# Nobita421/signature-Gan

Measured on AMD Instinct MI355X. Metric: signature images/sec (G+D train step, bs64 64x64 z=100), higher is better.
Workload: dtype f32; 1 GPU; configs[1]: reference conv G/D 64x64x1, z=100, batch 64 per GPU, f32, n_critic=1; global_batch=64, parallelism=dp1

## Files before the change

include/siggan.h:

```cpp
#ifndef SIGGAN_H
#define SIGGAN_H

#include <stddef.h>
#include <stdint.h>

#ifdef __cplusplus
extern "C" {
#endif

#define SIGGAN_ABI_VERSION 4

enum {
    SIGGAN_OK = 0,
    SIGGAN_E_INVALID = -1,
    SIGGAN_E_STATE = -2,
    SIGGAN_E_HIP = -3,
    SIGGAN_E_NOMEM = -4
};

typedef struct siggan_ctx siggan_ctx;

typedef struct siggan_config {
    int32_t device;
    int32_t latent_dim;
// ... 40 lines not shown

int64_t siggan_param_count(const siggan_ctx *ctx, int which);
int32_t siggan_param_tensors(const siggan_ctx *ctx, int which);
int siggan_param_span(const siggan_ctx *ctx, int which, int32_t idx, int64_t *offset, int64_t *numel);
int64_t siggan_bn_count(const siggan_ctx *ctx);
int64_t siggan_sn_count(const siggan_ctx *ctx, int which);
int32_t siggan_bn_layers(const siggan_ctx *ctx);
int64_t siggan_workspace_bytes(const siggan_ctx *ctx);

int siggan_bind(siggan_ctx *ctx, const siggan_storage *st);
int siggan_params_changed(siggan_ctx *ctx);
int siggan_seed(siggan_ctx *ctx, uint64_t seed, uint64_t offset);
int siggan_rng_state(siggan_ctx *ctx, uint64_t *seed, uint64_t *offset);
#define SIGGAN_MODE_GRAPH 1
#define SIGGAN_MODE_OVERLAP 2
int siggan_set_mode(siggan_ctx *ctx, int32_t mode);

enum { SIGGAN_STEP_TRAINER = 0, SIGGAN_STEP_ABLATION = 1 };
int siggan_set_step_variant(siggan_ctx *ctx, int32_t variant);

int siggan_g_forward(siggan_ctx *ctx, const float *z_dev, int32_t batch, int32_t training,
                     float *images_dev, void *stream);

enum { SIGGAN_IS_NEG = 0, SIGGAN_IS_INK_SIGNED = 1, SIGGAN_IS_INK_UNIT = 2, SIGGAN_IS_COUNT = 3 };
int siggan_g_generate_u8(siggan_ctx *ctx, const float *z_dev, int32_t batch, uint8_t *u8_dev,
                         float *images_dev, int32_t *stats_dev, float threshold, void *stream);

int siggan_g_latent_grad(siggan_ctx *ctx, const float *z_dev, int32_t batch, const uint8_t *target_u8_dev,
                         const float *target_f32_dev, float *dz_dev, float *loss_dev, float *images_dev, void *stream);

// ... 83 lines not shown
```

signature-gan_amd/csrc/ctx.h:

```cpp
#pragma once
#include <hip/hip_runtime.h>
#include <dlfcn.h>
#include <math.h>
#include <stdarg.h>
#include <stdio.h>
#include <stdlib.h>
#include <string.h>
#include <new>
#include <vector>

#include "../../include/siggan.h"
#include "gconv.h"
#include "host.h"
#include "ops.h"

using namespace siggan;

static const float BN_MOMENTUM = 0.1f, BN_EPS = 1e-5f;
static const int MAXL = 6;
static const int64_t PARTIAL_FLOATS = (int64_t)2 << 20;
static const float SN_EPS = 1e-12f;
#define EV_FLAGS (hipEventDisableTiming | hipEventDisableSystemFence)
#define LAUNCHCHK()                                                                                 \
    do {                                                                                            \
        hipError_t e_ = hipGetLastError();                                                          \
        if (e_ != hipSuccess) return FAIL(SIGGAN_E_HIP, "kernel launch -> %s (%s:%d)", hipGetErrorString(e_), __FILE__, __LINE__); \
    } while (0)
#define ENTER(c)                                                     \
    if (!(c)) return FAIL(SIGGAN_E_INVALID, "null context");          \
    DevGuard dg_((c)->cfg.device);                                    \
    HIPCHK(dg_.err)

typedef struct ncclComm* ncclComm_t;
typedef struct { char internal[128]; } ncclUniqueId_t;
enum { NCCL_SUCCESS = 0, NCCL_CHAR = 0, NCCL_FLOAT32 = 7, NCCL_SUM = 0 };
struct Rccl {
// ... 178 lines not shown
    void refuse(const char* why) { c->refused = why; }
    void comm_fail(int rc) { c->comm_err = rc; }
    void record(hipEvent_t e, hipStream_t s) { note(hipEventRecord(e, s)); }
    void wait(hipStream_t s, hipEvent_t e) { note(hipStreamWaitEvent(s, e, 0)); }
};

struct WgradCall { WgradArgs w; int max_splits; };
struct BceSpec { int n0; float y0, y1; float* mt; int is_g; };
struct GFwdOpt {
    bool training = false;
    float *partial = nullptr, *slab_k = nullptr;
    uint32_t rng_sid = 0; float* z_out = nullptr;
    hipEvent_t done = nullptr;
    uint8_t* u8 = nullptr; int32_t* stats = nullptr; float thr = 0.f;
    bool keep_y = false;
};
struct DFwdOpt {
    bool dropout = false;
    bool fuse_cls = false;
    bool conv1_done = false;
    const uint8_t* u8 = nullptr; int binarize = -1; float* x_out = nullptr;
};

namespace siggan {
void drop_dreal(siggan_ctx* c);
int settle(siggan_ctx* c, hipStream_t s);
void invalidate(siggan_ctx* c, Inval why);
int check_bn_batch(const siggan_ctx* c, int batch);
int check_call(siggan_ctx* c, int batch, bool need_bound = true);
int lane_check(siggan_ctx* c);
// ... 16 lines not shown
```

signature-gan_amd/csrc/eval.hip:

```cpp
#include "ctx.h"

static int begin_eval(siggan_ctx* c, hipStream_t s, bool with_d, bool sn_power_iteration) {
    if (with_d) invalidate(c, INV_ROWS);
    const int rc = settle(c, s);
    if (rc) return rc;
    Lanes L(c, s);
    if (with_d) {
        if (c->sn) launch_sn_sigma(c->snt, sn_power_iteration, 2, SN_EPS, s);
        repack(c, L, s, s, c->g_dirty, c->sn || c->d_dirty, 2);
        c->g_dirty = c->d_dirty = false;
    } else {
        repack(c, L, s, s, c->g_dirty, !c->sn && c->d_dirty);
        c->g_dirty = false; if (!c->sn) c->d_dirty = false;
    }
    return SIGGAN_OK;
}

extern "C" int siggan_g_forward(siggan_ctx* c, const float* z_dev, int32_t batch, int32_t training, float* images_dev,
                                void* stream) {
    ENTER(c);
    int rc = check_call(c, batch);
    if (rc) return rc;
    if (training && (rc = check_bn_batch(c, batch))) return rc;
    if (!z_dev || !images_dev) return FAIL(SIGGAN_E_INVALID, "null tensor");
    hipStream_t s = (hipStream_t)stream;
    if ((rc = begin_eval(c, s, false, false))) return rc;
    GFwdOpt o; o.training = training != 0;
    c->cs.ga_last_B = g_forward_pass(c, z_dev, batch, images_dev, s, o);
    if (training) c->g_dirty = true;
    LAUNCHCHK();
    return lane_check(c);
}

extern "C" int siggan_g_generate_u8(siggan_ctx* c, const float* z_dev, int32_t batch, uint8_t* u8_dev, float* images_dev,
                                    int32_t* stats_dev, float threshold, void* stream) {
    ENTER(c);
    int rc = check_call(c, batch);
    if (rc) return rc;
    if (!z_dev || !u8_dev) return FAIL(SIGGAN_E_INVALID, "null tensor");
    if (reinterpret_cast<uintptr_t>(u8_dev) & 3) return FAIL(SIGGAN_E_INVALID, "u8_dev must be 4-byte aligned");
    if (stats_dev && !isfinite(threshold)) return FAIL(SIGGAN_E_INVALID, "threshold must be finite");
    hipStream_t s = (hipStream_t)stream;
// ... 208 lines not shown
```

signature-gan_amd/csrc/extras.hip:

```cpp
#include "ctx.h"

static bool pow2(int v) { return v > 0 && (v & (v - 1)) == 0; }

extern "C" int siggan_op_conv4x4s2(siggan_ctx* c, int32_t form, const void* in_dev, const float* w_dev, void* out_dev,
                                   int32_t batch, int32_t h_in, int32_t c_in, int32_t c_out, void* stream) {
    if (!c) return FAIL(SIGGAN_E_INVALID, "null context");
    if (!in_dev || !w_dev || !out_dev) return FAIL(SIGGAN_E_INVALID, "null tensor");
    if (form != 0 && form != 1) return FAIL(SIGGAN_E_INVALID, "form must be 0 (down) or 1 (up)");
    if (!pow2(h_in) || !pow2(c_in) || !pow2(c_out) || c_in < 32 || c_out < 32 || c_in > 512 || c_out > 512 || batch < 1)
        return FAIL(SIGGAN_E_INVALID, "shape not in the model family (pow2 dims, 32 <= C <= 512)");
    if (form == 0 && h_in < 2) return FAIL(SIGGAN_E_INVALID, "down form needs h_in >= 2");
    DevGuard dg_(c->cfg.device); HIPCHK(dg_.err);
    hipStream_t s = (hipStream_t)stream;
    GConvArgs a = gconv_args(c, form, batch, h_in, c_in, c_out);
    a.in = in_dev; a.wp = c->op_pack; a.out = out_dev; a.epi = EPI_RAW;
    PrepTable t; t.njobs = 0; t.overflow = 0;
    PrepJob j; memset(&j, 0, sizeof j);
    j.src = w_dev; j.dst = (float*)c->op_pack; j.dt = c->dt;
    if (form == 0) { j.type = PREP_PACK_DOWN; j.O = c_out; j.I = c_in; }
    else           { j.type = PREP_PACK_UP; j.I = c_in; j.O = c_out; }
    prep_add(t, j);
    if (!launch_prepare(t, BN_EPS, s)) return FAIL(SIGGAN_E_STATE, "prepare table overflow");
    launch_gconv(a, s);
    LAUNCHCHK();
// ... 129 lines not shown
    for (auto& r : g_prof_store.recs) {
        if (r.id != idx) continue;
        float t = 0.f;
        HIPCHK(hipEventElapsedTime(&t, r.e0, r.e1));
        *launches += 1; *ms += t; *flops += r.flops; *bytes += r.bytes;
    }
    return SIGGAN_OK;
}

extern "C" int siggan_prof_launch(siggan_ctx* c, int64_t idx, int32_t* fields, int32_t n, int64_t* count) {
    if (!c || !count || (n > 0 && !fields)) return FAIL(SIGGAN_E_INVALID, "bad argument");
    *count = (int64_t)g_prof_store.recs.size();
    if (n <= 0) return SIGGAN_OK;
    if (idx < 0 || idx >= *count) return FAIL(SIGGAN_E_INVALID, "launch %lld of %lld", (long long)idx, (long long)*count);
    const Prof::Rec& r = g_prof_store.recs[(size_t)idx];
    const int32_t v[7] = {r.id, r.form, r.epi_req, r.epi, r.M, r.Ci, r.Co};
    for (int i = 0; i < n && i < 7; ++i) fields[i] = v[i];
    return SIGGAN_OK;
}

extern "C" int siggan_debug_tensor(siggan_ctx* c, const char* name, int32_t idx, float* out_dev, int64_t n, void* stream) {
    if (!c || !name || !out_dev || n < 1) return FAIL(SIGGAN_E_INVALID, "bad argument");
    const void* src = nullptr; int64_t capv = 0;
    const void** ptr = &src; int64_t* cap = &capv;
    bool typed = true;
    const int64_t Bm = c->Bm, Bd = 2 * Bm, SS = (int64_t)c->S * c->S;
    auto gsz = [&](int l) { const int64_t H = 4 << l; return Bm * H * H * c->gC[l]; };
    auto dsz = [&](int l) { const int64_t H = c->S >> l; return Bd * H * H * c->dC[l]; };
    const bool gl = idx >= 0 && idx <= c->Lg, dl = idx >= 1 && idx <= c->Ld;
    if (!strcmp(name, "g_y") && gl) { *ptr = c->g_y[idx]; *cap = gsz(idx); }
    else if (!strcmp(name, "g_a") && gl) { *ptr = c->g_a[idx]; *cap = gsz(idx); }
    else if (!strcmp(name, "g_da") && gl) { *ptr = c->g_da[idx]; *cap = gsz(idx); }
// ... 11 lines not shown
    else if (!strcmp(name, "probs")) { *ptr = c->probs; *cap = Bd; typed = false; }
    else if (!strcmp(name, "dlogit")) { *ptr = c->dlogit; *cap = Bd; typed = false; }
    else if (!strcmp(name, "d_noise") && dl) { *ptr = c->d_noise[idx]; *cap = Bd * c->dC[idx]; typed = false; }
    else if (!strcmp(name, "rode") || !strcmp(name, "pre_real") || !strcmp(name, "ride_late")) {
        if (n != 1) return FAIL(SIGGAN_E_INVALID, "debug scalar %s holds 1 float, %lld asked", name, (long long)n);
        DevGuard dg_(c->cfg.device); HIPCHK(dg_.err);
        HIPCHK(hipStreamSynchronize((hipStream_t)stream));
        const float v = !strcmp(name, "rode") ? (float)c->cs.g_rode : !strcmp(name, "pre_real") ? (float)c->cs.g_pre_real
                                                                                               : (float)__atomic_load_n(c->ride_late, __ATOMIC_ACQUIRE);
        HIPCHK(hipMemcpy(out_dev, &v, sizeof v, hipMemcpyHostToDevice));
        return SIGGAN_OK;
    }
    else return FAIL(SIGGAN_E_INVALID, "unknown debug tensor %s[%d]", name, idx);
    if (n > capv) return FAIL(SIGGAN_E_INVALID, "debug tensor %s[%d] holds %lld floats, %lld asked", name, idx, (long long)capv, (long long)n);
    DevGuard dg_(c->cfg.device); HIPCHK(dg_.err);
    if (!strcmp(name, "g_a") && idx == c->Lg && c->cs.ga_last_B) {
        const int64_t H = c->S;
        HIPCHK(hipDeviceSynchronize());
        launch_bn_relu(c->dt, c->g_y[idx], c->g_a[idx], (int64_t)c->cs.ga_last_B * H * H, c->gC[idx], c->g_bn[idx], c->cfg.g_leaky_slope,
                       (hipStream_t)stream);
        LAUNCHCHK();
    }
    if (typed && c->dt != DT_F32) { launch_to_f32(c->dt, src, out_dev, n, (hipStream_t)stream); LAUNCHCHK(); }
    else HIPCHK(hipMemcpyAsync(out_dev, src, (size_t)n * sizeof(float), hipMemcpyDeviceToDevice, (hipStream_t)stream));
    return SIGGAN_OK;
}

extern "C" int siggan_augment_batch(int32_t device, const uint8_t* cache_dev, int64_t n_images, const int32_t* index_dev,
                                    const int32_t* params_dev, const int16_t* tables_dev, const float* lut_dev, float* out_dev,
                                    int32_t batch, int32_t size, int32_t augment, int32_t fill, void* stream) {
// ... 33 lines not shown
```

signature-gan_amd/csrc/gconv.h:

```cpp
#pragma once
#include <hip/hip_runtime.h>
#include <stdint.h>
#include <vector>

#include "act.h"

namespace siggan {

enum Epilogue : int {
    EPI_RAW = 0,
    EPI_BIAS_LRELU_DROP,
    EPI_AFFINE_RELU,
    EPI_LRELU_BWD,
    EPI_BN_BWD_STATS,
};

struct GConvArgs {
    int dt;
    const void* in;
    const void* wp;
    void* out;
    int B, Hi, Wi, Ci, Co;
    int lgHr, lgWr;
    int Ho, Wo;
// ... 5 lines not shown
    const float* scale;
    const float* shift;
    const void* aref;
    const float* bnp;
    float* stat0;
    float* stat1;
    int64_t stat_cap;
    const float* cls_w;
    float* cls_part;
    float slope;
    float gslope;
    float* slab;
    int64_t slab_floats;
    size_t slab_stride;
    const float* zeros;
};

struct BnBwdParams { f32x4 sc, sf, mu, rs; };
__device__ __forceinline__ BnBwdParams bn_bwd_params(const float* __restrict__ bnp, int Co, int co) {
    BnBwdParams q;
    q.sc = *reinterpret_cast<const f32x4*>(bnp + co); q.sf = *reinterpret_cast<const f32x4*>(bnp + Co + co);
    q.mu = *reinterpret_cast<const f32x4*>(bnp + 2 * Co + co); q.rs = *reinterpret_cast<const f32x4*>(bnp + 3 * Co + co);
    return q;
}
template <class T, bool LK>
__device__ __forceinline__ void bn_bwd_stat_terms(const f32x4 v, const f32x4 y, const BnBwdParams& q, float gs, f32x4& s0, f32x4& s1) {
#pragma unroll
    for (int e = 0; e < 4; ++e) {
        const float vq = (float)(T)v[e];
        const float d = g_dact<LK>(fmaf(y[e], q.sc[e], q.sf[e]), vq, gs);
// ... 11 lines not shown
    const void* L;
    float* slab;
    float* dw;
    float* db;
    int B, Cs, Cl;
    int lgHs, lgWs, lgCl;
    int K;
    int kchunk;
    const float* zeros;
};

struct Prof {
    struct Rec {
        int id; double flops, bytes; hipEvent_t e0, e1;
        int form, epi_req, epi, M, Ci, Co;
    };
    static constexpr int NID = 8;
    std::vector<Rec> recs;
    static const char* name(int id);
    void begin(int id, double flops, double bytes, hipStream_t st);
    void shape(const GConvArgs& a, int epi_req);
    void clear();
};
extern Prof* g_prof;

int launch_gconv(const GConvArgs& a, hipStream_t st);
void launch_gconv16(int cfg, const GConvArgs& a, dim3 grid, hipStream_t st, hipEvent_t e0, hipEvent_t e1, int kq = 1);
void launch_wgrad16(bool small, const WgradArgs& a, dim3 grid, hipStream_t st, hipEvent_t e0, hipEvent_t e1);
int launch_wgrad(WgradArgs a, int max_splits, hipStream_t st);

}
```

signature-gan_amd/csrc/gconv.hip:

```cpp
#include "gconv_parts.h"
#include "host.h"
#include <hip/hip_ext.h>

namespace siggan {

static constexpr int PAD = 4;

template <int BM, int BN, int WM, int WN, int KQ = 1, bool LK = false>
__global__ __launch_bounds__(256 * KQ) void k_gconv(const GConvArgs a) {
    constexpr int TM = BM / (32 * WM), TN = BN / (32 * WN);
    constexpr int PA = BM / 32, PB = BN / 32;
    constexpr int LD = BK + 4;
    __shared__ __attribute__((aligned(16))) float smem[KQ * 2 * LD * (BM + BN)];
    const GconvBlock<BM, BN, KQ> b(a);
    const int nk = b.nk;
    float* const sA = smem + b.quad * (2 * LD * (BM + BN));
    float* const sB = sA + 2 * LD * BM;

    const int lane = b.tid & 63, wave = b.tid >> 6;
    const int li = lane & 31, lh = lane >> 5;
    const int wm = wave / WN, wn = wave % WN;
    const float* const a_wp = static_cast<const float*>(a.wp);

    const int kc = b.tid & 7, rloc = b.tid >> 3;
// ... 120 lines not shown
            opix = (size_t)m;
        } else {
            const int rh = (m >> a.lgWr) & (b.Hr - 1), rw = m & (b.Wr - 1);
            opix = ((size_t)n * a.Ho + 2 * rh + b.ph) * a.Wo + 2 * rw + b.pw;
        }
        const size_t o = opix * a.Co + co;
        const f32x4 v = epi_apply<float, LK>(a, q, *reinterpret_cast<const f32x4*>(sT + row * LDT + c4 * 4), o, n, co);
        *reinterpret_cast<f32x4*>(outp + o) = v;
    }
    if (q.stats) {
        __syncthreads();
        epi_stats_reduce(a, q, sT, b.tid, b.quad == 0, c4, r0, C4, RPP, (size_t)b.cls * (gridDim.x / b.tiles_n) + b.bid / b.tiles_n, co);
    }
}

template <int CI, bool LK>
__global__ __launch_bounds__(256) void k_gconv_up4(const GConvArgs a) {
    constexpr int BM = 128, BN = 32, LD = BK + 4, LP = CI + 4, NCC = CI / BK;
    constexpr int PATCH_PIX = 264;
    constexpr int SMEM = (PATCH_PIX * LP + 2 * 4 * BN * LD) > (BM * 4 * BN) ? (PATCH_PIX * LP + 2 * 4 * BN * LD) : (BM * 4 * BN);
    __shared__ __attribute__((aligned(16))) float smem[SMEM];
    float* const sP = smem;
    float* const sB = smem + PATCH_PIX * LP;
    const int tid = threadIdx.x, lane = tid & 63, wave = tid >> 6;
    const int li = lane & 31, lh = lane >> 5;
    const int m0 = xcd_remap(blockIdx.x, gridDim.x) * BM;
    const int Hr = 1 << a.lgHr, Wr = 1 << a.lgWr, Wp = Wr + 2;
    const int Ktot = 4 * CI;
    const int n_img = m0 >> (a.lgHr + a.lgWr), rh0 = (m0 >> a.lgWr) & (Hr - 1), rows = BM >> a.lgWr;

    {
        const float* const img = static_cast<const float*>(a.in) + (size_t)n_img * a.Hi * a.Wi * CI;
        const int nchunk = (rows + 2) * Wp * (CI / 4);
        constexpr int NI = (PATCH_PIX * (CI / 4) + 255) / 256;
        f32x4 v[NI];
// ... 34 lines not shown
    };

    f32x16 acc[4];
#pragma unroll
    for (int cls = 0; cls < 4; ++cls)
#pragma unroll
        for (int r = 0; r < 16; ++r) acc[cls][r] = 0.f;

    load_tile();
    store_tile(0);
    load_tile();
    __syncthreads();

    const int ml = wave * 32 + li;
    const float* const pP = sP + (((ml >> a.lgWr) + 1) * Wp + (ml & (Wr - 1)) + 1) * LP + 4 * lh;

#pragma unroll
    for (int cls = 0; cls < 4; ++cls) {
        const int ph = cls >> 1, pw = cls & 1;
        for (int cc = 0; cc < NCC; ++cc) {
            const int kt = cls * NCC + cc, buf = kt & 1;
            const float* pA[4];
#pragma unroll
            for (int t = 0; t < 4; ++t) pA[t] = pP + ((ph - (t >> 1)) * Wp + (pw - (t & 1))) * LP + cc * BK;
            const float* pB = sB + (buf * 4 * BN + li) * LD + 4 * lh;
            f32x4 fa[2][4], fb[2][4];
#pragma unroll
            for (int t = 0; t < 4; ++t) {
                fa[0][t] = *reinterpret_cast<const f32x4*>(pA[t]);
                fb[0][t] = *reinterpret_cast<const f32x4*>(pB + t * BN * LD);
            }
#pragma unroll
            for (int c = 0; c < BK / 8; ++c) {
                const int cur = c & 1, nxt = cur ^ 1;
                if (c + 1 < BK / 8) {
#pragma unroll
                    for (int t = 0; t < 4; ++t) {
                        fa[nxt][t] = *reinterpret_cast<const f32x4*>(pA[t] + 8 * (c + 1));
                        fb[nxt][t] = *reinterpret_cast<const f32x4*>(pB + t * BN * LD + 8 * (c + 1));
                    }
                }
                __builtin_amdgcn_sched_barrier(0);
#pragma unroll
                for (int t = 0; t < 4; ++t)
#pragma unroll
                    for (int u = 0; u < 4; ++u)
                        acc[cls] = __builtin_amdgcn_mfma_f32_32x32x2f32(fa[cur][t][u], fb[cur][t][u], acc[cls], 0, 0, 0);
                if (c == 0 && kt + 1 < 4 * NCC) store_tile(buf ^ 1);
                if (c == 1 && kt + 2 < 4 * NCC) load_tile();
            }
            __syncthreads();
        }
    }

    const float sc = a.epi == EPI_AFFINE_RELU ? a.scale[li] : 1.f, sf = a.epi == EPI_AFFINE_RELU ? a.shift[li] : 0.f;
    const int Wo = 2 * Wr;
    float* const so = smem;
#pragma unroll
    for (int r = 0; r < 16; ++r) {
        const int mr = wave * 32 + (r & 3) + 8 * (r >> 2) + 4 * lh;
        const int rl = mr >> a.lgWr, rw = mr & (Wr - 1);
#pragma unroll
        for (int cls = 0; cls < 4; ++cls) {
            float v = acc[cls][r];
            if (a.epi == EPI_AFFINE_RELU) v = g_act<LK>(fmaf(v, sc, sf), a.gslope);
            so[(((2 * rl + (cls >> 1)) * Wo) + 2 * rw + (cls & 1)) * BN + li] = v;
        }
    }
    __syncthreads();
    f32x4* const dst = reinterpret_cast<f32x4*>(static_cast<float*>(a.out) + ((size_t)n_img * a.Ho + 2 * rh0) * a.Wo * BN);
    const f32x4* const src = reinterpret_cast<const f32x4*>(so);
#pragma unroll
// ... 34 lines not shown
        if ((threadIdx.x & 63) == 0) shc[threadIdx.x >> 6] = d;
        __syncthreads();
        if (threadIdx.x == 0) a.cls_part[blockIdx.x] = ((shc[0] + shc[1]) + shc[2]) + shc[3];
    }
}

Prof* g_prof = nullptr;

const char* Prof::name(int id) {
    static const char* n[NID] = {"k_gconv<128,128>", "k_gconv<128,64>", "k_gconv<64,64>", "k_gconv<128,32>",
                                 "k_wgrad<64,64>", "k_gconv_up4", "k_wgrad<32,128>", "?"};
    return n[id < 0 || id >= NID ? NID - 1 : id];
}
void Prof::begin(int id, double flops, double bytes, hipStream_t) {
    Rec r; r.id = id; r.flops = flops; r.bytes = bytes;
    r.form = r.epi_req = r.epi = r.M = r.Ci = r.Co = -1;
    (void)hipEventCreate(&r.e0); (void)hipEventCreate(&r.e1);
    recs.push_back(r);
}
void Prof::shape(const GConvArgs& a, int epi_req) {
    Rec& r = recs.back();
    r.form = a.form; r.epi_req = epi_req; r.epi = a.epi; r.M = a.M; r.Ci = a.Ci; r.Co = a.Co;
}
void Prof::clear() {
    for (auto& r : recs) { (void)hipEventDestroy(r.e0); (void)hipEventDestroy(r.e1); }
    recs.clear();
}

static double gconv_bytes(const GConvArgs& a) {
    const double es = (double)dt_size(a.dt);
    const double in = (double)a.B * a.Hi * a.Wi * a.Ci, out = (double)a.B * a.Ho * a.Wo * a.Co, w = 16.0 * a.Ci * a.Co;
// ... 31 lines not shown
    if (a.dt != DT_F32) {
        launch_gconv16(id, a, grid, st, e0, e1, KQ);
    } else if (gen_lk(a)) {
        hipExtLaunchKernelGGL((k_gconv<BM, BN, WM, WN, KQ, true>), grid, dim3(256 * KQ), 0, st, e0, e1, 0, a);
    } else if (g_prof) {
        hipExtLaunchKernelGGL((k_gconv<BM, BN, WM, WN, KQ>), grid, dim3(256 * KQ), 0, st, e0, e1, 0, a);
    } else {
        hipLaunchKernelGGL((k_gconv<BM, BN, WM, WN, KQ>), grid, dim3(256 * KQ), 0, st, a);
    }
    if (nsplit > 1)
        SIGGAN_GS_SWITCH(gen_lk(a) ? 1.f : 0.f, LK, SIGGAN_DT_SWITCH(a.dt, T, hipLaunchKernelGGL((k_splitk_epilogue<T, LK>),
            dim3((unsigned)((total4 + 255) / 256)), dim3(256), 0, st, a, nsplit, total4)));
    return rows;
}

int launch_gconv(const GConvArgs& a_in, hipStream_t st) {
    GConvArgs a = a_in;
    if (a.epi == EPI_BN_BWD_STATS && (a.stat0 == nullptr || a.stat_cap <= 0)) return -1;
    const int ncls = a.form == 0 ? 1 : 4;
    auto blocks = [&](int bm, int bn) { return ((a.M + bm - 1) / bm) * (a.Co / bn) * ncls; };
    const int nk = (a.form == 0 ? 16 : 4) * (a.Ci / BK);
    auto splits = [&](int nblk) {
        int ns = 1;
        if (a.slab && nblk < 384) {
            ns = (512 + nblk - 1) / nblk;
            if (ns > nk / 4) ns = nk / 4;
            if (ns > 8) ns = 8;
            const int64_t out_floats = (int64_t)a.B * a.Ho * a.Wo * a.Co;
            if (ns > 1 && (int64_t)ns * out_floats > a.slab_floats) ns = (int)(a.slab_floats / out_floats);
            if (ns < 1) ns = 1;
        }
        a.slab_stride = (size_t)a.B * a.Ho * a.Wo * a.Co;
        return ns;
    };
    if (a.Co >= 64) {
        if (a.Co >= 128 && blocks(128, 128) >= 512) return launch_cfg<128, 128, 2, 2>(a, st, 0, 1);
        const int ns = splits(blocks(64, 64));
        if (ns == 2 && (nk & 1) == 0) return launch_cfg<64, 64, 2, 2, 2>(a, st, 2, 1);
        if (ns == 4 && !a.cls_w && a.dt != DT_F32 && (nk & 1) == 0) return launch_cfg<64, 64, 2, 2, 2>(a, st, 2, 1);
        return launch_cfg<64, 64, 2, 2>(a, st, 2, ns);
    }
    if (a.dt == DT_F32 && a.form == 1 && a.Co == 32 && (a.epi == EPI_RAW || a.epi == EPI_AFFINE_RELU) && (a.Ci == 32 || a.Ci == 64) &&
        a.M / 128 >= (a.Ci == 32 ? 384 : 768) && a.M % 128 == 0 &&
        ((1 << (a.lgHr + a.lgWr)) % 128) == 0 && a.lgWr >= 4 && a.lgWr <= 6) {
        dim3 grid(a.M / 128);
        if (g_prof) {
            g_prof->begin(5, 2.0 * a.M * a.Co * (double)(4 * a.Ci) * 4, gconv_bytes(a), st);
            g_prof->shape(a, a.epi);
        }
        hipEvent_t e0 = g_prof ? g_prof->recs.back().e0 : nullptr, e1 = g_prof ? g_prof->recs.back().e1 : nullptr;
        if (gen_lk(a)) {
            if (a.Ci == 32) hipExtLaunchKernelGGL((k_gconv_up4<32, true>), grid, dim3(256), 0, st, e0, e1, 0, a);
            else hipExtLaunchKernelGGL((k_gconv_up4<64, true>), grid, dim3(256), 0, st, e0, e1, 0, a);
        } else {
            if (a.Ci == 32) hipExtLaunchKernelGGL((k_gconv_up4<32, false>), grid, dim3(256), 0, st, e0, e1, 0, a);
            else hipExtLaunchKernelGGL((k_gconv_up4<64, false>), grid, dim3(256), 0, st, e0, e1, 0, a);
        }
        return 0;
    }
    const int ns = splits(blocks(128, 32));
    return launch_cfg<128, 32, 4, 1>(a, st, 3, ns);
}

template <int BM, int BN, int WM, int WN>
__global__ __launch_bounds__(256) void k_wgrad(const WgradArgs a) {
    constexpr int TM = BM / (32 * WM), TN = BN / (32 * WN);
// ... 213 lines not shown
```

signature-gan_amd/csrc/passes.hip:

```cpp
#include "ctx.h"

static const float* sn_inv_sigma(const siggan_ctx* c, int slot, int layer) {
    return c->sn ? c->sn_sig + (slot * 2 + 1) * SnTable::MAXS + layer : nullptr;
}
static void prep_table(const siggan_ctx* c, int which, int sn_slot, PrepTable& t) {
    t.njobs = 0; t.overflow = 0;
    const float* P = which == 0 ? c->st.g_params : c->st.d_params;
    for (int kind : {DV_FC, DV_CONV, DV_T16, DV_BN, DV_TAPS})
        for (const Derived& r : c->rec[which]) {
            if (r.kind != kind || !r.dst) continue;
            PrepJob j; memset(&j, 0, sizeof j);
            j.src = P + r.off; j.dst = r.dst;
            if (which == 1) j.mul = sn_inv_sigma(c, sn_slot, r.layer - 1);
            if (kind == DV_CONV) {
                j.dt = c->dt;
                PrepJob up = j;
                j.type = PREP_PACK_DOWN; j.O = r.A; j.I = r.Bc;
                up.type = PREP_PACK_UP; up.I = r.A; up.O = r.Bc; up.dst = r.dst2;
                prep_add(t, which == 0 ? up : j);
                prep_add(t, which == 0 ? j : up);
                continue;
            }
            if (kind == DV_FC) { j.type = PREP_FC_T; j.O = r.A; j.I = r.Bc; }
            else if (kind == DV_T16) { j.type = PREP_CLS; j.O = r.A; }
// ... 57 lines not shown
WgradCall siggan::wgrad_args(const siggan_ctx* c, const void* small, const void* large, float* dw, float* slab, int B, int h_small,
                            int c_small, int c_large) {
    WgradCall g; memset(&g, 0, sizeof g);
    WgradArgs& w = g.w;
    w.zeros = c->zeros; w.dt = c->dt;
    w.S = small; w.L = large; w.slab = slab; w.dw = dw; w.B = B; w.Cs = c_small; w.Cl = c_large;
    w.lgHs = w.lgWs = ilog2(h_small); w.lgCl = ilog2(c_large); w.K = B * h_small * h_small;
    g.max_splits = (int)(c->slab_floats / ((int64_t)c_small * (16 * c_large + 1)));
    return g;
}

int siggan::g_forward_pass(const siggan_ctx* c, const float* z, int B, float* img, hipStream_t s, const GFwdOpt& o) {
    float* const partial = o.partial ? o.partial : c->partial;
    char* const* const A = o.training ? c->g_a : c->g_ae;
    const float gs = c->cfg.g_leaky_slope;
    if (c->fc_fused && launch_fc_fwd_fused(c->dt, z, GP(c, gi_fc_w()), GP(c, gi_fc_b()), c->fc_y, A[0], GP(c, gi_bn0_w()),
                                          GP(c, gi_bn0_b()), c->st.g_bn_running_mean, c->st.g_bn_running_var, c->st.g_bn_batches,
                                          c->g_bn[0], o.training ? nullptr : c->g_bne[0], o.z_out, c->dev, o.rng_sid, B, c->latent,
                                          c->gC[0], BN_MOMENTUM, BN_EPS, gs, s)) {
    } else if (!o.training) {
        launch_fc_fwd(c->dt, z, c->wfc_t, GP(c, gi_fc_b()), A[0], B, c->latent, c->gC[0], gs, s, c->g_bne[0], c->dev, o.rng_sid, o.z_out);
    } else {
        launch_fc_fwd(c->dt, z, c->wfc_t, GP(c, gi_fc_b()), c->fc_y, B, c->latent, c->gC[0], gs, s, nullptr, c->dev, o.rng_sid, o.z_out);
        launch_bn_train_stats(c->dt, c->fc_y, B, c->F, GP(c, gi_bn0_w()), GP(c, gi_bn0_b()), c->st.g_bn_running_mean,
                              c->st.g_bn_running_var, c->st.g_bn_batches, c->g_bn[0], partial, c->gC[0], BN_MOMENTUM,
                              BN_EPS, s);
        launch_bn_relu(c->dt, c->fc_y, A[0], B, c->F, c->g_bn[0], gs, s);
    }
    for (int l = 1; l <= c->Lg; ++l) {
        const int Hi = 4 << (l - 1), C = c->gC[l];
// ... 3 lines not shown
        const int64_t off = c->g_bn_off[l];
        if (o.training) {
            a.out = c->g_y[l]; a.epi = EPI_RAW;
            launch_gconv(a, s);
            const int64_t R = (int64_t)B * 4 * Hi * Hi;
            launch_bn_train_stats(c->dt, c->g_y[l], R, C, GP(c, gi_bn_w(l)), GP(c, gi_bn_b(l)), c->st.g_bn_running_mean + off,
                                  c->st.g_bn_running_var + off, c->st.g_bn_batches + l, c->g_bn[l], partial, 0,
                                  BN_MOMENTUM, BN_EPS, s);
            if (l < c->Lg) launch_bn_relu(c->dt, c->g_y[l], A[l], R, C, c->g_bn[l], gs, s);
        } else if (o.keep_y) {
            a.out = c->g_y[l]; a.epi = EPI_RAW;
            launch_gconv(a, s);
            launch_bn_relu(c->dt, c->g_y[l], A[l], (int64_t)B * 4 * Hi * Hi, C, c->g_bne[l], gs, s);
        } else {
            a.out = A[l]; a.epi = EPI_AFFINE_RELU; a.scale = c->g_bne[l]; a.shift = c->g_bne[l] + C;
            launch_gconv(a, s);
        }
    }
    if (o.training)
        launch_final_fwd(c->dt, c->g_y[c->Lg], c->wfin_t, GP(c, gi_fin_b(c)), img, B, c->S, c->gC[c->Lg], gs, s, c->g_bn[c->Lg], o.done);
    else
        launch_final_fwd(c->dt, A[c->Lg], c->wfin_t, GP(c, gi_fin_b(c)), img, B, c->S, c->gC[c->Lg], gs, s, nullptr, o.done, o.u8, o.stats, o.thr);
    return o.training ? B : 0;
}

int siggan::d_forward_rows(const siggan_ctx* c, const float* x, int r0, int nB, hipStream_t s, float* slab_k, const DFwdOpt& o) {
    const float slope = c->cfg.leaky_slope;
    int P = 0;
    auto act = [&](int l) { const int64_t H = c->S >> l; return c->d_a[l] + (size_t)((int64_t)r0 * H * H * c->dC[l]) * c->es; };
    auto nz = [&](int l) { return o.dropout ? c->d_noise[l] + (int64_t)r0 * c->dC[l] : nullptr; };
    if (o.u8)
        launch_conv1_fwd_u8(c->dt, Conv1U8{o.u8, c->deq_lut, o.x_out, o.binarize}, c->sn ? c->d_w1s : DP(c, di_w(1)), DP(c, di_b(1)), slope,
                            act(1), nB, c->S, c->dC[1], s);
// ... 163 lines not shown
```

signature-gan_amd/csrc/siggan.hip:

```cpp
#include "ctx.h"

static thread_local char g_err[512] = "";
int siggan_set_error(int code, const char* fmt, ...) {
    va_list ap;
    va_start(ap, fmt);
    vsnprintf(g_err, sizeof g_err, fmt, ap);
    va_end(ap);
    return code;
}

extern "C" int siggan_abi_version(void) { return SIGGAN_ABI_VERSION; }
extern "C" const char* siggan_last_error(void) { return g_err; }

static void build_layout(siggan_ctx* c) {
    static const int g64[] = {256, 128, 64, 32, 32}, g128[] = {512, 256, 128, 64, 32, 32};
    static const int d64[] = {1, 64, 128, 256, 512}, d128[] = {1, 64, 128, 256, 512, 512};
    if (c->S == 64) { c->Lg = 4; c->Ld = 4; memcpy(c->gC, g64, sizeof g64); memcpy(c->dC, d64, sizeof d64); }
    else            { c->Lg = 5; c->Ld = 5; memcpy(c->gC, g128, sizeof g128); memcpy(c->dC, d128, sizeof d128); }
    c->F = c->gC[0] * 16;
    c->g_bn_off[0] = 0; c->bn_total = c->F;
    for (int l = 1; l <= c->Lg; ++l) { c->g_bn_off[l] = c->bn_total; c->bn_total += c->gC[l]; }
    c->g_total = c->d_total = 0;
    auto rec = [c](int w, int kind, int layer, int64_t n, int64_t n2, int A = 0, int Bc = 0) {
        auto& off = w == 0 ? c->g_off : c->d_off;
// ... 343 lines not shown
    if (c->lane_err == hipSuccess) return SIGGAN_OK;
    const hipError_t e = c->lane_err; c->lane_err = hipSuccess;
    return FAIL(SIGGAN_E_HIP, "an event record / stream wait / prepare table of the step failed: %s", hipGetErrorString(e));
}

extern "C" int siggan_set_step_variant(siggan_ctx* c, int32_t variant) {
    if (!c) return FAIL(SIGGAN_E_INVALID, "null context");
    if (variant != SIGGAN_STEP_TRAINER && variant != SIGGAN_STEP_ABLATION) return FAIL(SIGGAN_E_INVALID, "unknown step variant %d", variant);
    if (c->cs.g_fwd_pending || c->cs.pending) return FAIL(SIGGAN_E_STATE, "a step is in flight");
    c->variant = variant;
    return SIGGAN_OK;
}

extern "C" int siggan_set_mode(siggan_ctx* c, int32_t mode) {
    if (!c) return FAIL(SIGGAN_E_INVALID, "null context");
    c->mode = mode;
    return SIGGAN_OK;
}

extern "C" int siggan_device_info(int32_t device, int32_t* compute_units, int32_t* clock_khz, int64_t* hbm_bytes) {
    if (!compute_units || !clock_khz || !hbm_bytes) return FAIL(SIGGAN_E_INVALID, "null argument");
    hipDeviceProp_t p;
    HIPCHK(hipGetDeviceProperties(&p, device));
    *compute_units = p.multiProcessorCount; *clock_khz = p.clockRate; *hbm_bytes = (int64_t)p.totalGlobalMem;
    return SIGGAN_OK;
}
```

signature-gan_amd/csrc/step.hip:

```cpp
#include "ctx.h"

int siggan::check_hyper(const siggan_hyper* hp) {
    if (!hp) return FAIL(SIGGAN_E_INVALID, "null hyper-parameters");
    if (!(hp->lr >= 0.0) || !(hp->beta1 >= 0.0 && hp->beta1 < 1.0) || !(hp->beta2 >= 0.0 && hp->beta2 < 1.0) || !(hp->eps >= 0.0))
        return FAIL(SIGGAN_E_INVALID, "invalid Adam hyper-parameters");
    return SIGGAN_OK;
}

static void phase_d_grads_sn(const siggan_ctx* c, Lanes& L, const PhaseKey& k, PhaseResult& r) {
    const int B = k.B;
    const bool drop = c->cfg.dropout > 0.f;
    repack(c, L, L.m, L.m, k.g_dirty != 0, false);
    if (k.pre_real)
        L.note(hipMemcpyAsync(c->real_stage, k.staged_src, (size_t)B * c->S * c->S * sizeof(float), hipMemcpyDeviceToDevice, L.m));
    if (drop) make_noise(c, k.has_masks ? c->mask_stage : nullptr, B, 0, 2, L.m);
    const float* fake = c->img;
    GFwdOpt ge, gt;
    ge.rng_sid = 1; ge.z_out = c->z; gt.training = true; gt.rng_sid = 2; gt.z_out = c->z_g;
    if (k.variant == SIGGAN_STEP_ABLATION) {
        r.ga_last_B = g_forward_pass(c, k.has_zg ? c->z_g : nullptr, B, c->img_g, L.m, gt);
        L.record(c->ev_gfwd, L.m);
        fake = c->img_g;
    } else {
        r.ga_last_B = g_forward_pass(c, k.has_z ? c->z : nullptr, B, c->img, L.m, ge);
    }
    DFwdOpt fo; fo.dropout = drop;
    launch_sn_sigma(c->snt, 1, 0, SN_EPS, L.m);
    repack(c, L, L.m, L.m, false, true, 0);
    r.lP[0] = d_forward_rows(c, c->real_stage, 0, B, L.m, c->slab_k, fo);
    launch_sn_sigma(c->snt, 1, 1, SN_EPS, L.m);
    repack(c, L, L.m, L.m, false, true, 1);
    r.lP[1] = d_forward_rows(c, fake, B, B, L.m, c->slab_k, fo);
    launch_bce(LogitSrc{c->logits}, 2 * B, B, k.ls, 0.f, c->probs, c->dlogit, k.mt, 0, L.m, c->gscale);
// ... 2 lines not shown
    d_backward_pass(c, L, c->real_stage, B, c->real_stage, B, drop, true, false, BceSpec{B, k.ls, k.ls, nullptr, 0}, r.lP[0], 0, c->sn_g[0]);
    SnTable t = c->snt;
    t.slot[0] = 0; t.slot[1] = 1;
    launch_sn_combine(t, c->sn_g[0], c->sn_g[1], c->st.d_grads, c->d_total, 2, L.m);
}

static void phase_d_grads(const siggan_ctx* c, Lanes& L, const PhaseKey& k, PhaseResult& r) {
    r.early_ar = 0;
    if (c->sn) return phase_d_grads_sn(c, L, k, r);
    const int B = k.B;
    const bool drop = c->cfg.dropout > 0.f;
    const bool nolane = k.pre_real == 2 && !k.d_dirty && (!drop || k.dreal_noise2);
    DFwdOpt fo; fo.dropout = drop; fo.fuse_cls = true;
    GFwdOpt ge, gt;
    ge.rng_sid = 1; ge.z_out = c->z; gt.training = true; gt.rng_sid = 2; gt.z_out = c->z_g;
    const float* xreal = c->real_stage;
    int P_real = k.lP0;
    if (nolane) {
        repack(c, L, L.m, L.m, k.g_dirty != 0, false);
        xreal = k.staged_src;
    } else {
    L.fork(L.a);
    repack(c, L, L.m, L.a, k.g_dirty != 0, k.d_dirty != 0);
    if (k.pre_real)
        L.note(hipMemcpyAsync(c->real_stage, k.staged_src, (size_t)B * c->S * c->S * sizeof(float), hipMemcpyDeviceToDevice, L.a));
    if (drop && !(k.pre_real == 2 && k.dreal_noise2))
        make_noise(c, k.has_masks ? c->mask_stage : nullptr, B, k.pre_real == 2 ? 1 : 0, 2, L.a);
    if (k.pre_real != 2) r.lP[0] = P_real = d_forward_rows(c, c->real_stage, 0, B, L.a, c->slab_k2, fo);
    }
    const float* fake = c->img;
// ... 414 lines not shown
```

signature-gan_amd/engine.py:

```python
import ctypes as C
import math

import torch

from . import _lib, layout


def _ptr(t):
    return C.c_void_p(t.data_ptr()) if t is not None else C.c_void_p(0)


def _f32(t, device, what):
    if t is None:
        return None
    if t.device != device:
        raise ValueError(f"{what} must live on {device}, got {t.device}")
    if t.dtype != torch.float32:
        raise ValueError(f"{what} must be float32, got {t.dtype}")
    return t.contiguous()


def check_objective_weights(recon_weight, realism_weight, prior_weight, has_target, want_probs=False, seeded=False):
    w = (float(recon_weight), float(realism_weight), float(prior_weight))
    if any(not math.isfinite(x) or x < 0.0 for x in w):
# ... 138 lines not shown
        for which in ("g", "d"):
            for k, v in self.views(which).items():
                if k.endswith("bias"):
                    v.zero_()
                else:
                    mean = 1.0 if ".1.weight" in k else 0.0
                    v.copy_(torch.empty(v.shape).normal_(mean, 0.02, generator=gen))
            for a in ("grads", "exp_avg", "exp_avg_sq", "adam_steps"):
                getattr(self, f"{which}_{a}").zero_()
        self.g_bn_mean.zero_(); self.g_bn_var.fill_(1.0); self.g_bn_batches.zero_()
        self.params_changed()

    def params_changed(self):
        _lib.check(self.lib.siggan_params_changed(self._h))

    def set_mode(self, graph=False, overlap=True):
        self._mode = (1 if graph else 0) | (2 if overlap else 0)
        _lib.check(self.lib.siggan_set_mode(self._h, self._mode))

    def set_step_variant(self, variant="trainer"):
        v = {"trainer": 0, "ablation": 1}[variant]
        _lib.check(self.lib.siggan_set_step_variant(self._h, v))
        self.step_variant = variant

    def ablation_step(self, real, z=None, masks=None, lr_d=2e-4, lr_g=2e-4, beta1=0.5, beta2=0.999, eps=1e-8,
                      label_smoothing=0.9, sync=True):
        if getattr(self, "step_variant", "trainer") != "ablation":
            raise RuntimeError("call set_step_variant('ablation') first")
        self.d_compute_grads(real, z, masks, label_smoothing, mask_passes=3)
        dm = self.d_apply(lr_d, beta1, beta2, eps, None, 1.0, sync)
        self.g_compute_grads(real.shape[0], label_smoothing=label_smoothing)
        gm = self.g_apply(lr_g, beta1, beta2, eps, None, 1.0, sync)
# ... 406 lines not shown
            _lib.check(self.lib.siggan_prof_read(self._h, i, name, 64, C.byref(n), C.byref(ms), C.byref(fl), C.byref(by)))
            if n.value:
                out.append({"name": name.value.decode(), "launches": n.value, "ms": ms.value, "flops": fl.value,
                            "bytes": by.value})
        return out

    def prof_launches(self):
        names = {}
        for i in range(self.lib.siggan_prof_slots()):
            buf = C.create_string_buffer(64)
            n, ms, fl, by = C.c_int64(), C.c_double(), C.c_double(), C.c_double()
            _lib.check(self.lib.siggan_prof_read(self._h, i, buf, 64, C.byref(n), C.byref(ms), C.byref(fl), C.byref(by)))
            names[i] = buf.value.decode()
        count = C.c_int64()
        _lib.check(self.lib.siggan_prof_launch(self._h, 0, None, 0, C.byref(count)))
        f = (C.c_int32 * 7)()
        out = []
        for i in range(count.value):
            _lib.check(self.lib.siggan_prof_launch(self._h, i, f, 7, C.byref(count)))
            epi = lambda e: _lib.EPILOGUES[e] if 0 <= e < len(_lib.EPILOGUES) else None
            out.append({"kernel": names.get(f[0], "?"), "form": f[1], "epi_req": epi(f[2]), "epi": epi(f[3]), "M": f[4],
                        "Ci": f[5], "Co": f[6]})
        return out

    def debug_tensor(self, name, index, shape):
        n = 1
        for s in shape:
            n *= s
        out = torch.empty(n, dtype=torch.float32, device=self.device)
        _lib.check(self.lib.siggan_debug_tensor(self._h, name.encode(), index, _ptr(out), n, self._stream()))
        return out.view(shape)

    def close(self):
        self._staged = None
        if getattr(self, "_h", None):
            self.lib.siggan_destroy(self._h)
            self._h = None
# ... 7 lines not shown
```

Baseline: 45370 images/s.

## Fuse generator final 3x3 conv and tanh into last up-conv kernel for eval forward

```diff
diff --git a/include/siggan.h b/include/siggan.h
--- a/include/siggan.h
+++ b/include/siggan.h
@@ -78,6 +78,7 @@
 int siggan_rng_state(siggan_ctx *ctx, uint64_t *seed, uint64_t *offset);
 #define SIGGAN_MODE_GRAPH 1
 #define SIGGAN_MODE_OVERLAP 2
+#define SIGGAN_MODE_SPLIT_TAIL 4
 int siggan_set_mode(siggan_ctx *ctx, int32_t mode);
 
 enum { SIGGAN_STEP_TRAINER = 0, SIGGAN_STEP_ABLATION = 1 };
diff --git a/signature-gan_amd/csrc/ctx.h b/signature-gan_amd/csrc/ctx.h
--- a/signature-gan_amd/csrc/ctx.h
+++ b/signature-gan_amd/csrc/ctx.h
@@ -20,6 +20,7 @@
 static const int MAXL = 6;
 static const int64_t PARTIAL_FLOATS = (int64_t)2 << 20;
 static const float SN_EPS = 1e-12f;
+static const int GA_UNWRITTEN = 1 << 30;
 #define EV_FLAGS (hipEventDisableTiming | hipEventDisableSystemFence)
 #define LAUNCHCHK()                                                                                 \
     do {                                                                                            \
@@ -228,6 +229,7 @@
     hipEvent_t done = nullptr;
     uint8_t* u8 = nullptr; int32_t* stats = nullptr; float thr = 0.f;
     bool keep_y = false;
+    bool fuse_tail = false;
 };
 struct DFwdOpt {
     bool dropout = false;
diff --git a/signature-gan_amd/csrc/eval.hip b/signature-gan_amd/csrc/eval.hip
--- a/signature-gan_amd/csrc/eval.hip
+++ b/signature-gan_amd/csrc/eval.hip
@@ -26,6 +26,7 @@
     hipStream_t s = (hipStream_t)stream;
     if ((rc = begin_eval(c, s, false, false))) return rc;
     GFwdOpt o; o.training = training != 0;
+    o.fuse_tail = !o.training;
     c->cs.ga_last_B = g_forward_pass(c, z_dev, batch, images_dev, s, o);
     if (training) c->g_dirty = true;
     LAUNCHCHK();
diff --git a/signature-gan_amd/csrc/extras.hip b/signature-gan_amd/csrc/extras.hip
--- a/signature-gan_amd/csrc/extras.hip
+++ b/signature-gan_amd/csrc/extras.hip
@@ -167,8 +167,8 @@
     if (n <= 0) return SIGGAN_OK;
     if (idx < 0 || idx >= *count) return FAIL(SIGGAN_E_INVALID, "launch %lld of %lld", (long long)idx, (long long)*count);
     const Prof::Rec& r = g_prof_store.recs[(size_t)idx];
-    const int32_t v[7] = {r.id, r.form, r.epi_req, r.epi, r.M, r.Ci, r.Co};
-    for (int i = 0; i < n && i < 7; ++i) fields[i] = v[i];
+    const int32_t v[8] = {r.id, r.form, r.epi_req, r.epi, r.M, r.Ci, r.Co, r.tail};
+    for (int i = 0; i < n && i < 8; ++i) fields[i] = v[i];
     return SIGGAN_OK;
 }
 
@@ -210,6 +210,9 @@
     else return FAIL(SIGGAN_E_INVALID, "unknown debug tensor %s[%d]", name, idx);
     if (n > capv) return FAIL(SIGGAN_E_INVALID, "debug tensor %s[%d] holds %lld floats, %lld asked", name, idx, (long long)capv, (long long)n);
     DevGuard dg_(c->cfg.device); HIPCHK(dg_.err);
+    if (!strcmp(name, "g_a") && idx == c->Lg && (c->cs.ga_last_B & GA_UNWRITTEN))
+        return FAIL(SIGGAN_E_STATE, "debug tensor g_a[%d]: the last Generator forward formed the image inside its last block and did not "
+                                    "write that activation (SIGGAN_MODE_SPLIT_TAIL keeps the two launches)", idx);
     if (!strcmp(name, "g_a") && idx == c->Lg && c->cs.ga_last_B) {
         const int64_t H = c->S;
         HIPCHK(hipDeviceSynchronize());
diff --git a/signature-gan_amd/csrc/gconv.h b/signature-gan_amd/csrc/gconv.h
--- a/signature-gan_amd/csrc/gconv.h
+++ b/signature-gan_amd/csrc/gconv.h
@@ -43,6 +43,9 @@
     int64_t slab_floats;
     size_t slab_stride;
     const float* zeros;
+    const float* fin_w;
+    const float* fin_b;
+    float* fin_img;
 };
 
 struct BnBwdParams { f32x4 sc, sf, mu, rs; };
@@ -84,6 +87,7 @@
     struct Rec {
         int id; double flops, bytes; hipEvent_t e0, e1;
         int form, epi_req, epi, M, Ci, Co;
+        int tail;
     };
     static constexpr int NID = 8;
     std::vector<Rec> recs;
@@ -94,7 +98,8 @@
 };
 extern Prof* g_prof;
 
-int launch_gconv(const GConvArgs& a, hipStream_t st);
+int launch_gconv(const GConvArgs& a, hipStream_t st, hipEvent_t done = nullptr);
+bool gconv_fuses_tail(const GConvArgs& a);
 void launch_gconv16(int cfg, const GConvArgs& a, dim3 grid, hipStream_t st, hipEvent_t e0, hipEvent_t e1, int kq = 1);
 void launch_wgrad16(bool small, const WgradArgs& a, dim3 grid, hipStream_t st, hipEvent_t e0, hipEvent_t e1);
 int launch_wgrad(WgradArgs a, int max_splits, hipStream_t st);
diff --git a/signature-gan_amd/csrc/gconv.hip b/signature-gan_amd/csrc/gconv.hip
--- a/signature-gan_amd/csrc/gconv.hip
+++ b/signature-gan_amd/csrc/gconv.hip
@@ -158,11 +158,12 @@
     }
 }
 
-template <int CI, bool LK>
+template <int CI, bool LK, bool FT = false>
 __global__ __launch_bounds__(256) void k_gconv_up4(const GConvArgs a) {
     constexpr int BM = 128, BN = 32, LD = BK + 4, LP = CI + 4, NCC = CI / BK;
     constexpr int PATCH_PIX = 264;
-    constexpr int SMEM = (PATCH_PIX * LP + 2 * 4 * BN * LD) > (BM * 4 * BN) ? (PATCH_PIX * LP + 2 * 4 * BN * LD) : (BM * 4 * BN);
+    constexpr int OUT_FLOATS = FT ? (8 + 2) * 64 * BN : BM * 4 * BN;
+    constexpr int SMEM = (PATCH_PIX * LP + 2 * 4 * BN * LD) > OUT_FLOATS ? (PATCH_PIX * LP + 2 * 4 * BN * LD) : OUT_FLOATS;
     __shared__ __attribute__((aligned(16))) float smem[SMEM];
     float* const sP = smem;
     float* const sB = smem + PATCH_PIX * LP;
@@ -227,6 +228,13 @@
 
     const int ml = wave * 32 + li;
     const float* const pP = sP + (((ml >> a.lgWr) + 1) * Wp + (ml & (Wr - 1)) + 1) * LP + 4 * lh;
+    const int hw = __builtin_amdgcn_readfirstlane(wave);
+    const int hrow = hw >> 1, hcls = hrow ? (hw & 1) : 2 + (hw & 1);
+    const bool hlive = FT && (hrow ? rh0 + rows < Hr : rh0 > 0);
+    const int dH = FT ? (int)((sP + ((hrow ? rows + 1 : 0) * Wp + li + 1) * LP + 4 * lh) - pP) : 0;
+    f32x16 acch;
+#pragma unroll
+    for (int r = 0; r < 16; ++r) acch[r] = 0.f;
 
 #pragma unroll
     for (int cls = 0; cls < 4; ++cls) {
@@ -253,12 +261,25 @@
                         fb[nxt][t] = *reinterpret_cast<const f32x4*>(pB + t * BN * LD + 8 * (c + 1));
                     }
                 }
+                const bool halo = FT && hlive && cls == hcls;
+                f32x4 fh[4];
+                if (halo) {
+#pragma unroll
+                    for (int t = 0; t < 4; ++t) fh[t] = *reinterpret_cast<const f32x4*>(pA[t] + dH + 8 * c);
+                }
                 __builtin_amdgcn_sched_barrier(0);
 #pragma unroll
                 for (int t = 0; t < 4; ++t)
 #pragma unroll
                     for (int u = 0; u < 4; ++u)
                         acc[cls] = __builtin_amdgcn_mfma_f32_32x32x2f32(fa[cur][t][u], fb[cur][t][u], acc[cls], 0, 0, 0);
+                if (halo) {
+#pragma unroll
+                    for (int t = 0; t < 4; ++t)
+#pragma unroll
+                        for (int u = 0; u < 4; ++u)
+                            acch = __builtin_amdgcn_mfma_f32_32x32x2f32(fh[t][u], fb[cur][t][u], acch, 0, 0, 0);
+                }
                 if (c == 0 && kt + 1 < 4 * NCC) store_tile(buf ^ 1);
                 if (c == 1 && kt + 2 < 4 * NCC) load_tile();
             }
@@ -269,6 +290,56 @@
     const float sc = a.epi == EPI_AFFINE_RELU ? a.scale[li] : 1.f, sf = a.epi == EPI_AFFINE_RELU ? a.shift[li] : 0.f;
     const int Wo = 2 * Wr;
     float* const so = smem;
+    if (FT) {
+        const int c4 = tid & 7, px = tid >> 3;
+        f32x4 w[9];
+#pragma unroll
+        for (int k = 0; k < 9; ++k) w[k] = *reinterpret_cast<const f32x4*>(a.fin_w + k * 32 + c4 * 4);
+        const float bias = a.fin_b[0];
+#pragma unroll
+        for (int r = 0; r < 16; ++r) {
+            const int mr = wave * 32 + (r & 3) + 8 * (r >> 2) + 4 * lh;
+            const int rl = mr >> 5, rw = mr & 31;
+#pragma unroll
+            for (int cls = 0; cls < 4; ++cls)
+                so[(((1 + 2 * rl + (cls >> 1)) * 64) + 2 * rw + (cls & 1)) * BN + li] = g_act<LK>(fmaf(acc[cls][r], sc, sf), a.gslope);
+            const int hx = 2 * ((r & 3) + 8 * (r >> 2) + 4 * lh) + (hw & 1);
+            so[((hrow ? 9 : 0) * 64 + hx) * BN + li] = hlive ? g_act<LK>(fmaf(acch[r], sc, sf), a.gslope) : 0.f;
+        }
+        __syncthreads();
+        float* const orow = a.fin_img + ((size_t)n_img * a.Ho + 2 * rh0) * a.Wo;
+#pragma unroll
+        for (int h = 0; h < 2; ++h) {
+            const int x = 32 * h + px;
+            const float* const pl = so + (x > 0 ? x - 1 : 0) * BN + c4 * 4;
+            const float* const pc = so + x * BN + c4 * 4;
+            const float* const pr = so + (x < 63 ? x + 1 : 63) * BN + c4 * 4;
+            const f32x4 z4 = {0.f, 0.f, 0.f, 0.f};
+            f32x4 v[3][3];
+            float mine = 0.f;
+#pragma unroll
+            for (int r = 0; r < 8 + 2; ++r) {
+                const f32x4 ql = *reinterpret_cast<const f32x4*>(pl + r * 64 * BN), qr = *reinterpret_cast<const f32x4*>(pr + r * 64 * BN);
+                v[r % 3][0] = x > 0 ? ql : z4;
+                v[r % 3][1] = *reinterpret_cast<const f32x4*>(pc + r * 64 * BN);
+                v[r % 3][2] = x < 63 ? qr : z4;
+                if (r < 2) continue;
+                const int y = r - 2;
+                float s = 0.f;
+#pragma unroll
+                for (int kh = 0; kh < 3; ++kh)
+#pragma unroll
+                    for (int kw = 0; kw < 3; ++kw) {
+                        const f32x4 av = v[(y + kh) % 3][kw], ww = w[kh * 3 + kw];
+                        s = fmaf(av.x, ww.x, s); s = fmaf(av.y, ww.y, s); s = fmaf(av.z, ww.z, s); s = fmaf(av.w, ww.w, s);
+                    }
+                s += __shfl_xor(s, 4, 8); s += __shfl_xor(s, 2, 8); s += __shfl_xor(s, 1, 8);
+                mine = c4 == y ? s : mine;
+            }
+            orow[c4 * a.Wo + x] = tanhf(mine + bias);
+        }
+        return;
+    }
 #pragma unroll
     for (int r = 0; r < 16; ++r) {
         const int mr = wave * 32 + (r & 3) + 8 * (r >> 2) + 4 * lh;
@@ -333,7 +404,7 @@
 }
 void Prof::begin(int id, double flops, double bytes, hipStream_t) {
     Rec r; r.id = id; r.flops = flops; r.bytes = bytes;
-    r.form = r.epi_req = r.epi = r.M = r.Ci = r.Co = -1;
+    r.form = r.epi_req = r.epi = r.M = r.Ci = r.Co = -1; r.tail = 0;
     (void)hipEventCreate(&r.e0); (void)hipEventCreate(&r.e1);
     recs.push_back(r);
 }
@@ -395,7 +466,17 @@
     return rows;
 }
 
-int launch_gconv(const GConvArgs& a_in, hipStream_t st) {
+static bool up4_ok(const GConvArgs& a) {
+    return a.dt == DT_F32 && a.form == 1 && a.Co == 32 && (a.epi == EPI_RAW || a.epi == EPI_AFFINE_RELU) && (a.Ci == 32 || a.Ci == 64) &&
+           a.M / 128 >= (a.Ci == 32 ? 384 : 768) && a.M % 128 == 0 &&
+           ((1 << (a.lgHr + a.lgWr)) % 128) == 0 && a.lgWr >= 4 && a.lgWr <= 6;
+}
+bool gconv_fuses_tail(const GConvArgs& a) {
+    return a.fin_img != nullptr && a.fin_w != nullptr && a.fin_b != nullptr && up4_ok(a) && a.Ci == 32 && a.epi == EPI_AFFINE_RELU &&
+           a.lgWr == 5 && a.lgHr == 5;
+}
+
+int launch_gconv(const GConvArgs& a_in, hipStream_t st, hipEvent_t done) {
     GConvArgs a = a_in;
     if (a.epi == EPI_BN_BWD_STATS && (a.stat0 == nullptr || a.stat_cap <= 0)) return -1;
     const int ncls = a.form == 0 ? 1 : 4;
@@ -421,16 +502,23 @@
         if (ns == 4 && !a.cls_w && a.dt != DT_F32 && (nk & 1) == 0) return launch_cfg<64, 64, 2, 2, 2>(a, st, 2, 1);
         return launch_cfg<64, 64, 2, 2>(a, st, 2, ns);
     }
-    if (a.dt == DT_F32 && a.form == 1 && a.Co == 32 && (a.epi == EPI_RAW || a.epi == EPI_AFFINE_RELU) && (a.Ci == 32 || a.Ci == 64) &&
-        a.M / 128 >= (a.Ci == 32 ? 384 : 768) && a.M % 128 == 0 &&
-        ((1 << (a.lgHr + a.lgWr)) % 128) == 0 && a.lgWr >= 4 && a.lgWr <= 6) {
+    if (up4_ok(a)) {
         dim3 grid(a.M / 128);
+        const bool tail = gconv_fuses_tail(a);
         if (g_prof) {
-            g_prof->begin(5, 2.0 * a.M * a.Co * (double)(4 * a.Ci) * 4, gconv_bytes(a), st);
+            const double out = (double)a.B * a.Ho * a.Wo;
+            g_prof->begin(5, 2.0 * a.M * a.Co * (double)(4 * a.Ci) * 4,
+                          tail ? gconv_bytes(a) - 4.0 * out * a.Co + 4.0 * (out + 9.0 * a.Co + 1.0) : gconv_bytes(a), st);
             g_prof->shape(a, a.epi);
+            g_prof->recs.back().tail = tail;
         }
         hipEvent_t e0 = g_prof ? g_prof->recs.back().e0 : nullptr, e1 = g_prof ? g_prof->recs.back().e1 : nullptr;
-        if (gen_lk(a)) {
+        if (tail) {
+            if (!e1) e1 = done;
+            if (gen_lk(a)) hipExtLaunchKernelGGL((k_gconv_up4<32, true, true>), grid, dim3(256), 0, st, e0, e1, 0, a);
+            else hipExtLaunchKernelGGL((k_gconv_up4<32, false, true>), grid, dim3(256), 0, st, e0, e1, 0, a);
+            if (done && e1 != done) (void)hipEventRecord(done, st);
+        } else if (gen_lk(a)) {
             if (a.Ci == 32) hipExtLaunchKernelGGL((k_gconv_up4<32, true>), grid, dim3(256), 0, st, e0, e1, 0, a);
             else hipExtLaunchKernelGGL((k_gconv_up4<64, true>), grid, dim3(256), 0, st, e0, e1, 0, a);
         } else {
diff --git a/signature-gan_amd/csrc/passes.hip b/signature-gan_amd/csrc/passes.hip
--- a/signature-gan_amd/csrc/passes.hip
+++ b/signature-gan_amd/csrc/passes.hip
@@ -95,6 +95,7 @@
     float* const partial = o.partial ? o.partial : c->partial;
     char* const* const A = o.training ? c->g_a : c->g_ae;
     const float gs = c->cfg.g_leaky_slope;
+    bool fused = false;
     if (c->fc_fused && launch_fc_fwd_fused(c->dt, z, GP(c, gi_fc_w()), GP(c, gi_fc_b()), c->fc_y, A[0], GP(c, gi_bn0_w()),
                                           GP(c, gi_bn0_b()), c->st.g_bn_running_mean, c->st.g_bn_running_var, c->st.g_bn_batches,
                                           c->g_bn[0], o.training ? nullptr : c->g_bne[0], o.z_out, c->dev, o.rng_sid, B, c->latent,
@@ -128,9 +129,14 @@
             launch_bn_relu(c->dt, c->g_y[l], A[l], (int64_t)B * 4 * Hi * Hi, C, c->g_bne[l], gs, s);
         } else {
             a.out = A[l]; a.epi = EPI_AFFINE_RELU; a.scale = c->g_bne[l]; a.shift = c->g_bne[l] + C;
-            launch_gconv(a, s);
-        }
-    }
+            if (l == c->Lg && o.fuse_tail && !o.u8 && (c->mode & SIGGAN_MODE_SPLIT_TAIL) == 0) {
+                a.fin_w = c->wfin_t; a.fin_b = GP(c, gi_fin_b(c)); a.fin_img = img;
+                fused = gconv_fuses_tail(a);
+            }
+            launch_gconv(a, s, fused ? o.done : nullptr);
+        }
+    }
+    if (fused) return GA_UNWRITTEN | B;
     if (o.training)
         launch_final_fwd(c->dt, c->g_y[c->Lg], c->wfin_t, GP(c, gi_fin_b(c)), img, B, c->S, c->gC[c->Lg], gs, s, c->g_bn[c->Lg], o.done);
     else
diff --git a/signature-gan_amd/csrc/siggan.hip b/signature-gan_amd/csrc/siggan.hip
--- a/signature-gan_amd/csrc/siggan.hip
+++ b/signature-gan_amd/csrc/siggan.hip
@@ -381,6 +381,12 @@
 
 extern "C" int siggan_set_mode(siggan_ctx* c, int32_t mode) {
     if (!c) return FAIL(SIGGAN_E_INVALID, "null context");
+    if (((c->mode ^ mode) & SIGGAN_MODE_SPLIT_TAIL) && !c->graphs.empty()) {
+        DevGuard dg_(c->cfg.device); HIPCHK(dg_.err);
+        HIPCHK(hipDeviceSynchronize());
+        for (auto& e : c->graphs) (void)hipGraphExecDestroy(e.exec);
+        c->graphs.clear();
+    }
     c->mode = mode;
     return SIGGAN_OK;
 }
diff --git a/signature-gan_amd/csrc/step.hip b/signature-gan_amd/csrc/step.hip
--- a/signature-gan_amd/csrc/step.hip
+++ b/signature-gan_amd/csrc/step.hip
@@ -17,6 +17,7 @@
     const float* fake = c->img;
     GFwdOpt ge, gt;
     ge.rng_sid = 1; ge.z_out = c->z; gt.training = true; gt.rng_sid = 2; gt.z_out = c->z_g;
+    ge.fuse_tail = true;
     if (k.variant == SIGGAN_STEP_ABLATION) {
         r.ga_last_B = g_forward_pass(c, k.has_zg ? c->z_g : nullptr, B, c->img_g, L.m, gt);
         L.record(c->ev_gfwd, L.m);
@@ -49,6 +50,7 @@
     DFwdOpt fo; fo.dropout = drop; fo.fuse_cls = true;
     GFwdOpt ge, gt;
     ge.rng_sid = 1; ge.z_out = c->z; gt.training = true; gt.rng_sid = 2; gt.z_out = c->z_g;
+    ge.fuse_tail = true;
     const float* xreal = c->real_stage;
     int P_real = k.lP0;
     if (nolane) {
diff --git a/signature-gan_amd/engine.py b/signature-gan_amd/engine.py
--- a/signature-gan_amd/engine.py
+++ b/signature-gan_amd/engine.py
@@ -176,8 +176,10 @@
     def params_changed(self):
         _lib.check(self.lib.siggan_params_changed(self._h))
 
-    def set_mode(self, graph=False, overlap=True):
-        self._mode = (1 if graph else 0) | (2 if overlap else 0)
+    def set_mode(self, graph=False, overlap=True, split_tail=None):
+        if split_tail is None:
+            split_tail = bool(self._mode & 4)
+        self._mode = (1 if graph else 0) | (2 if overlap else 0) | (4 if split_tail else 0)
         _lib.check(self.lib.siggan_set_mode(self._h, self._mode))
 
     def set_step_variant(self, variant="trainer"):
@@ -614,13 +616,13 @@
             names[i] = buf.value.decode()
         count = C.c_int64()
         _lib.check(self.lib.siggan_prof_launch(self._h, 0, None, 0, C.byref(count)))
-        f = (C.c_int32 * 7)()
+        f = (C.c_int32 * 8)()
         out = []
         for i in range(count.value):
-            _lib.check(self.lib.siggan_prof_launch(self._h, i, f, 7, C.byref(count)))
+            _lib.check(self.lib.siggan_prof_launch(self._h, i, f, 8, C.byref(count)))
             epi = lambda e: _lib.EPILOGUES[e] if 0 <= e < len(_lib.EPILOGUES) else None
             out.append({"kernel": names.get(f[0], "?"), "form": f[1], "epi_req": epi(f[2]), "epi": epi(f[3]), "M": f[4],
-                        "Ci": f[5], "Co": f[6]})
+                        "Ci": f[5], "Co": f[6], "fused_tail": bool(f[7])})
         return out
 
     def debug_tensor(self, name, index, shape):
```

After: 45680 images/s (median of 6 runs). About the same (+0.7%).
